# Lut99/RayTracer-3

Measured on AMD Instinct MI355X. Metric: Msamples/sec (pixels x spp) at 1920x1080x512spp, higher is better.
Workload: dtype f32

## Files before the change

include/rt3.h:

```cpp
#ifndef RT3_H
#define RT3_H

#include <stdint.h>

#ifdef __cplusplus
extern "C" {
#endif

#define RT3_ABI_VERSION 3u
uint32_t rt3_abi_version(void);


#define RT3_E_ARG     (-1)
#define RT3_E_DEVICE  (-2)
#define RT3_E_IO      (-3)
#define RT3_E_STATE   (-4)


typedef struct rt3_gface {
    uint32_t v1, v2, v3;
    uint32_t _pad0;
    float    normal[3];
    uint32_t _pad1;
    float    color[3];
// ... 237 lines not shown
uint32_t rt3_scene_weekend(uint32_t seed, float* center_radius, rt3_material* materials, uint32_t cap);
uint32_t rt3_scene_stress(uint32_t n, uint32_t seed, float* center_radius, rt3_material* materials, uint32_t cap);
uint32_t rt3_scene_cornell(uint32_t grid, rt3_gface* faces, float* vertices_xyzw, rt3_material* face_materials,
                           uint32_t cap_faces);

uint32_t rt3_hash_u32(uint32_t x);
float    rt3_random_float(uint32_t m);

int      rt3_debug_force_plain_mode_r(rt3_ctx* ctx, int on);
int      rt3_debug_force_brute(rt3_ctx* ctx, int on);
int      rt3_debug_force_flat_filter(rt3_ctx* ctx, int on);
int      rt3_debug_arith(rt3_ctx* ctx, const float* a, const float* b, uint32_t n, float* div, float* sq, float* fm,
                         float* cs, float* sn, float* sk3, uint32_t* pk);
int      rt3_debug_primary_lists(rt3_ctx* ctx, const rt3_camera* cam, const rt3_params* p, uint32_t* out_masks, uint64_t capacity_words,
                                 uint32_t* n_groups, uint32_t* n_blocks);

#ifdef __cplusplus
}
#endif
#endif
```

raytracer-3_amd/__init__.py:

```python
import ctypes as C
import os

import numpy as np

_HERE = os.path.dirname(os.path.abspath(__file__))
LIB_PATH = os.environ.get("RT3_LIB_PATH", os.path.join(_HERE, "librt3hip.so"))

GFACE = np.dtype([("v1", "<u4"), ("v2", "<u4"), ("v3", "<u4"), ("_p0", "<u4"),
                  ("normal", "<f4", 3), ("_p1", "<u4"), ("color", "<f4", 3), ("_p2", "<u4")])
MATERIAL = np.dtype([("rgb", "<f4", 3), ("param", "<f4"), ("kind", "<u4")])

MAT_FLAT, MAT_LAMBERT, MAT_METAL, MAT_DIELECTRIC = 0, 1, 2, 3
RAY = np.dtype([("origin", "<f4", 3), ("t_max", "<f4"), ("direction", "<f4", 3), ("_pad", "<u4")])
HIT = np.dtype([("t", "<f4"), ("kind", "<u4"), ("index", "<u4"), ("_pad", "<u4")])
HIT_NONE, HIT_FACE, HIT_SPHERE, HIT_INVALID = 0, 1, 2, 3
AOV = np.dtype([("albedo", "<f4", 3), ("coverage", "<f4"), ("normal", "<f4", 3), ("depth", "<f4"), ("kind", "<u4"), ("index", "<u4"),
                ("_pad", "<u4", 2)])
HISTORY = np.dtype([("colour", "<f4", 3), ("length", "<f4"), ("moments", "<f4", 2), ("depth", "<f4"), ("_pad0", "<f4"),
                    ("normal", "<f4", 3), ("_pad1", "<f4")])
OCCLUDED_INVALID = 0xFFFFFFFF
FLAG_GAMMA2, FLAG_BLACK_BACKGROUND, FLAG_REFERENCE_PRIMARY, FLAG_VARIANCE = 1, 2, 4, 8
REGROUP_SPHERES, REGROUP_MESH = 1, 2


# ... 73 lines not shown
    "rt3_render", "rt3_render_device", "rt3_render_path", "rt3_render_path_device", "rt3_rows_owned",
    "rt3_row_of_local", "rt3_get_stats", "rt3_prerender_triangle", "rt3_sphere_face_count",
    "rt3_sphere_vertex_count", "rt3_prerender_sphere", "rt3_object_count", "rt3_prerender_object",
    "rt3_transfer_entity", "rt3_camera_update", "rt3_camera_look_at", "rt3_frame_ppm_bytes", "rt3_frame_to_ppm",
    "rt3_scene_three_spheres", "rt3_scene_weekend", "rt3_scene_stress", "rt3_scene_cornell", "rt3_hash_u32",
    "rt3_random_float", "rt3_debug_arith", "rt3_debug_force_plain_mode_r",
    "rt3_mesh_begin", "rt3_mesh_put", "rt3_mesh_sphere", "rt3_mesh_commit", "rt3_mesh_download",
    "rt3_render_path_range", "rt3_render_path_range_device", "rt3_accum_download", "rt3_accum_upload", "rt3_gather_rows",
    "rt3_stream", "rt3_synchronize", "rt3_device_alloc_words", "rt3_device_free", "rt3_device_read_words", "rt3_debug_force_brute",
    "rt3_abi_version", "rt3_debug_force_flat_filter", "rt3_gather_plan",
    "rt3_intersect", "rt3_occluded", "rt3_intersect_device", "rt3_occluded_device",
    "rt3_camera_rays", "rt3_camera_rays_device", "rt3_render_aov", "rt3_render_aov_device", "rt3_accum_resolve", "rt3_accum_resolve_device",
    "rt3_frame_pfm_bytes", "rt3_frame_to_pfm", "rt3_denoise", "rt3_denoise_device", "rt3_denoise_temporal", "rt3_denoise_temporal_device",
    "rt3_motion", "rt3_motion_device", "rt3_denoise_temporal_motion", "rt3_denoise_temporal_motion_device",
    "rt3_update_spheres", "rt3_update_spheres_device", "rt3_update_mesh", "rt3_update_mesh_device",
    "rt3_debug_primary_lists",
    "rt3_regroup", "rt3_regroup_device", "rt3_debug_group_order",
    "rt3_render_path_adaptive", "rt3_render_path_adaptive_device",
]
ABI_VERSION = 3

_lib = None


def lib():
    global _lib
    if _lib is not None:
        return _lib
    if not os.path.exists(LIB_PATH):
        raise Fatal("librt3hip.so not found at %s — build it with `python -c 'import __graft_entry__ as g; g.build()'`; "
                    "there is no CPU fallback" % LIB_PATH)
# ... 11 lines not shown
        "rt3_render_path": (i32, [vp, vp, vp, vp]), "rt3_render_path_device": (i32, [vp, vp, vp, vp, vp]),
        "rt3_rows_owned": (u32, [vp]), "rt3_row_of_local": (u32, [vp, u32]), "rt3_get_stats": (i32, [vp, vp]),
        "rt3_prerender_triangle": (None, [vp, vp, vp, vp, vp, vp]),
        "rt3_sphere_face_count": (u32, [u32, u32]), "rt3_sphere_vertex_count": (u32, [u32, u32]),
        "rt3_prerender_sphere": (None, [vp, f32, u32, u32, vp, vp, vp]),
        "rt3_object_count": (i32, [C.c_char_p, vp, vp]),
        "rt3_prerender_object": (i32, [C.c_char_p, vp, f32, vp, vp, u32, vp, u32]),
        "rt3_transfer_entity": (None, [vp, vp, vp, vp, vp, u32, vp, u32]),
        "rt3_camera_update": (None, [vp, f32, f32, f32]), "rt3_camera_look_at": (None, [vp, vp, vp, vp, f32, f32, f32]),
        "rt3_frame_ppm_bytes": (u64, [vp, u32, u32, vp, u64]), "rt3_frame_to_ppm": (i32, [vp, u32, u32, C.c_char_p]),
        "rt3_scene_three_spheres": (u32, [vp, vp, u32]), "rt3_scene_weekend": (u32, [u32, vp, vp, u32]),
        "rt3_scene_stress": (u32, [u32, u32, vp, vp, u32]), "rt3_scene_cornell": (u32, [u32, vp, vp, vp, u32]),
        "rt3_hash_u32": (u32, [u32]), "rt3_random_float": (f32, [u32]),
        "rt3_debug_arith": (i32, [vp, vp, vp, u32, vp, vp, vp, vp, vp, vp, vp]),
        "rt3_debug_force_plain_mode_r": (i32, [vp, i32]),
        "rt3_debug_primary_lists": (i32, [vp, vp, vp, vp, u64, vp, vp]),
        "rt3_mesh_begin": (i32, [vp, u32, u32]), "rt3_mesh_put": (i32, [vp, vp, u32, vp, u32, u32, u32]),
        "rt3_mesh_sphere": (i32, [vp, vp, f32, u32, u32, vp, u32, u32]), "rt3_mesh_commit": (i32, [vp, vp]),
        "rt3_mesh_download": (i32, [vp, vp, vp]),
        "rt3_render_path_range": (i32, [vp, vp, vp, u32, u32, vp]),
        "rt3_render_path_range_device": (i32, [vp, vp, vp, u32, u32, vp, vp]),
        "rt3_accum_download": (i32, [vp, vp, vp, vp]), "rt3_accum_upload": (i32, [vp, vp, vp, vp, vp, u32]),
        "rt3_gather_rows": (i32, [vp, vp, vp, vp, vp, vp]), "rt3_stream": (vp, [vp]), "rt3_synchronize": (i32, [vp]),
        "rt3_device_alloc_words": (vp, [vp, u64]), "rt3_device_free": (None, [vp, vp]),
        "rt3_device_read_words": (i32, [vp, vp, u64, vp]), "rt3_debug_force_brute": (i32, [vp, i32]),
        "rt3_abi_version": (u32, []), "rt3_debug_force_flat_filter": (i32, [vp, i32]), "rt3_gather_plan": (i32, [vp, vp]),
        "rt3_intersect": (i32, [vp, vp, u32, f32, vp]), "rt3_occluded": (i32, [vp, vp, u32, f32, vp]),
        "rt3_intersect_device": (i32, [vp, vp, u32, f32, vp, vp]), "rt3_occluded_device": (i32, [vp, vp, u32, f32, vp, vp]),
        "rt3_camera_rays": (i32, [vp, vp, vp, u32, u32, vp]), "rt3_camera_rays_device": (i32, [vp, vp, vp, u32, u32, vp, vp]),
        "rt3_render_aov": (i32, [vp, vp, vp, vp]), "rt3_render_aov_device": (i32, [vp, vp, vp, vp, vp]),
        "rt3_accum_resolve": (i32, [vp, vp]), "rt3_accum_resolve_device": (i32, [vp, vp, vp]),
# ... 735 lines not shown
        return outs


    def debug_primary_lists(self, cam, params):
        ng, nb = C.c_uint32(0), C.c_uint32(0)
        npix = rows_owned(params) * params.width
        out = np.zeros((-(-npix // 64), 16), np.uint32)
        self._check(lib().rt3_debug_primary_lists(self._ctx, C.byref(cam), C.byref(params), _p(out), out.size, C.byref(ng), C.byref(nb)))
        return out.reshape(-1)[:ng.value * nb.value].reshape(ng.value, nb.value).copy()


def initialize_renderer(device=0):
    return HipRenderer(device)


def rows_owned(params):
    return lib().rt3_rows_owned(C.byref(params))


def row_of_local(params, local_row):
    return lib().rt3_row_of_local(C.byref(params), local_row)


def deinterleave(tiles, params_list, height, width):
    frame = np.zeros((height, width), np.uint32)
    for tile, p in zip(tiles, params_list):
        for r in range(tile.shape[0]):
            frame[row_of_local(p, r)] = tile[r]
    return frame
```

raytracer-3_amd/csrc/rt3_device.hip:

```cpp
#include <hip/hip_runtime.h>
#include <hipcub/hipcub.hpp>

#include <algorithm>
#include <cmath>
#include <cstdio>
#include <cstdlib>
#include <cstring>
#include <map>
#include <set>
#include <string>
#include <type_traits>
#include <vector>

#include "rt3.h"

#include "rt3_kernel_common.hpp"
#include "rt3_path.hpp"
#include "rt3_valu_scan.hpp"
#include "rt3_matrix_filter.hpp"
#include "rt3_level_filter.hpp"
#include "rt3_reduce.hpp"
#include "rt3_adaptive.hpp"
#include "rt3_aov.hpp"
#include "rt3_denoise.hpp"
// ... 517 lines not shown
    const bool sph_lds = has_sph && ctx->n_sph <= kSphLdsMax;
    const bool grouped = kGroupTri > 1 && kGroupSph > 1 && (query || (!ctx->force_flat && !getenv("RT3_NO_GROUPS")));
    A.n_tri_rows = grouped ? ctx->tri.n_groups : ctx->n_faces;
    A.n_sph_rows = grouped ? ctx->sph.n_groups : ctx->n_sph;
    A.sph_grp = ctx->sph.grp; A.sph_perm = ctx->sph.perm; A.tri_grp = ctx->tri.grp; A.tri_perm = ctx->tri.perm; A.tri_rec = ctx->d_tri_rec;
    A.tri_leaf = ctx->tri.leaf; A.sph_leaf = ctx->sph.leaf; A.n_tri_leaves = ctx->tri.n_leaves; A.n_sph_leaves = ctx->sph.n_leaves;
    A.tri_rowb = ctx->tri.rowb; A.sph_rowb = ctx->sph.rowb;
    T.mfma_blocks = (ctx->n_sph + 31u) / 32u;
    bool resident = false;
    uint32_t levels = 0;
    if (brute) {
        T.plain = query ? k_trace_brute<false, true> : ref ? k_trace_brute<true> : list ? k_trace_brute<false, false, true> : k_trace_brute<false>;
    } else if (mfma_single) {
        T.lds = single_k64 ? (size_t)T.mfma_blocks * (4096 + 32 * (16 + 16 + 4 + 4)) + (size_t)kBitmapBytes
                           : (size_t)T.mfma_blocks * (2048 + 32 * (16 + 16 + 4 + 4)) + (size_t)kBitmapBytes + (size_t)kMB * 8 + (size_t)(kMB / 64) * kPairCap * 4;
        T.block = kMB;
        T.single = single_k64 ? (list ? k_trace_mfma<true> : k_trace_mfma<>) : query ? k_trace_mfma32<true> : list ? k_trace_mfma32<false, true> : k_trace_mfma32<>;
        T.frag_a = (const u32x4*)(single_k64 ? ctx->d_sph_frag.get() : ctx->d_sph_frag32.get());
        if (!query && !single_k64) {
            T.filter_counted = true;
            const char* on = getenv("RT3_PRIMARY_LISTS"); const char* cap = getenv("RT3_PRIMARY_LIST_MAX");
            A.prim_masks = nullptr;
            A.prim_list_max = 0;
            if (!list && !(on && atoi(on) == 0)) {
                T.list_groups = (A.npix + 63u) / 64u;
                int rc_;
                if ((rc_ = ctx->d_prim_masks.ensure(ctx, (size_t)T.list_groups * T.mfma_blocks))) return rc_;
                A.prim_masks = ctx->d_prim_masks;
                A.prim_list_max = cap ? (uint32_t)std::min<long>(std::max<long>(atol(cap), 0), (long)kMfmaSphMax) : kPrimaryListMax;
            }
// ... 1514 lines not shown
    RT3_HIP(hipEventElapsedTime(&out->total_ms, ctx->ev_begin, ctx->ev_end));
    out->launches = ctx->ev_used;
    out->samples = ctx->last_samples;
    out->n_spheres = ctx->n_sph;
    out->n_faces = ctx->n_faces;
    if (ctx->last_was_path) {
        unsigned long long counters[kCastSlots] = { 0 };
        RT3_HIP(hipMemcpy(counters, ctx->d_casts, sizeof counters, hipMemcpyDeviceToHost));
#ifdef RT3_PROFILE_PHASES
        if (counters[13] != 0) {
            const double all = (double)(counters[11] + counters[12] + counters[13] + counters[14] + counters[15] + counters[17]);
            fprintf(stderr, "[rt3 profile] k_trace_mfma32 / k_trace_mfma, share of wave time: refill %.1f %%, ray operands (+ direct spheres) %.1f %%, scan %.1f %%, "
                            "push + exact tests %.1f %%, decode + shade %.1f %%, restock (primary pass) %.1f %%\n",
                    100.0 * counters[11] / all, 100.0 * counters[12] / all, 100.0 * counters[13] / all, 100.0 * counters[14] / all, 100.0 * counters[15] / all,
                    100.0 * counters[17] / all);
        }
#endif
#ifdef RT3_PROFILE
        if (counters[13] == 0)
        fprintf(stderr, "[rt3 profile] wave iterations %llu, flush iterations/wave-iter %.2f, candidates/ray %.2f, live lanes/wave-iter %.1f, "
                        "fresh paths/wave-iter %.1f\n", counters[4], (double)counters[2] / (double)counters[4],
                (double)counters[3] / (double)counters[0], (double)counters[0] / (double)counters[4], (double)counters[5] / (double)counters[4]);
        if (counters[13] != 0) {
            const double all = (double)(counters[12] + counters[13] + counters[14] + counters[15] + counters[4]);
            fprintf(stderr, "[rt3 profile] tiled kernel, share of wave time: barriers + tile fill %.1f %%, scan %.1f %%, push %.1f %%, exact tests %.1f %%, "
                            "refill / operands / shade %.1f %%\n", 100.0 * counters[12] / all, 100.0 * counters[13] / all, 100.0 * counters[14] / all,
                    100.0 * counters[15] / all, 100.0 * counters[4] / all);
        } else {
        fprintf(stderr, "[rt3 profile] first wave ended %.1f us before the last one\n", (double)(counters[7] - counters[6]) / 100.0);
        fprintf(stderr, "[rt3 profile] timeline from the first wave's start (us): last wave start %.1f, queue first seen empty %.1f, last seen empty %.1f, "
// ... 30 lines not shown
    RT3_HIP(hipMemcpy(da, a, N * 4, hipMemcpyHostToDevice));
    RT3_HIP(hipMemcpy(db, b, N * 4, hipMemcpyHostToDevice));
    hipLaunchKernelGGL(k_debug_arith, dim3((n + 255) / 256), dim3(256), 0, ctx->stream, da, db, n, ddiv, dsq, dfm, dcs, dsn, dsk, dpk);
    RT3_HIP(hipGetLastError());
    RT3_HIP(hipStreamSynchronize(ctx->stream));
    RT3_HIP(hipMemcpy(div, ddiv, N * 4, hipMemcpyDeviceToHost));
    RT3_HIP(hipMemcpy(sq, dsq, N * 4, hipMemcpyDeviceToHost));
    RT3_HIP(hipMemcpy(fm, dfm, N * 4, hipMemcpyDeviceToHost));
    RT3_HIP(hipMemcpy(cs, dcs, N * 4, hipMemcpyDeviceToHost));
    RT3_HIP(hipMemcpy(sn, dsn, N * 4, hipMemcpyDeviceToHost));
    RT3_HIP(hipMemcpy(sk3, dsk, N * 12, hipMemcpyDeviceToHost));
    RT3_HIP(hipMemcpy(pk, dpk, N * 4, hipMemcpyDeviceToHost));
    return 0;
}

int rt3_debug_primary_lists(rt3_ctx* ctx, const rt3_camera* cam, const rt3_params* p, uint32_t* out_masks, uint64_t capacity_words, uint32_t* n_groups,
                            uint32_t* n_blocks) {
    if (!ctx) return RT3_E_ARG;
    if (!cam || !n_groups || !n_blocks) return fail(ctx, RT3_E_ARG, "cam / n_groups / n_blocks is NULL");
    int rc = check_params(ctx, p);
    if (rc) return rc;
    if (ctx->n_sph == 0 || ctx->n_faces != 0 || ctx->n_sph > kMfmaSphMax) return fail(ctx, RT3_E_STATE, "strip lists need a sphere-only scene of <= 512 spheres");
    hipStream_t stream;
    if ((rc = enter(ctx, nullptr, &stream))) return rc;
    const uint32_t npix = rt3_rows_owned(p) * p->width;
    *n_groups = (npix + 63u) / 64u;
    *n_blocks = (ctx->n_sph + 31u) / 32u;
    const size_t words = (size_t)*n_groups * *n_blocks;
    if (!out_masks || capacity_words < words) return fail(ctx, RT3_E_ARG, "out_masks holds fewer than n_groups * n_blocks words");
    if (words == 0) return 0;
// ... 11 lines not shown
```

raytracer-3_amd/csrc/rt3_kernel_common.hpp:

```cpp
#pragma once

namespace {

constexpr int      kBlock       = 256;
constexpr int      kCandSlots   = 16;
constexpr uint32_t kWorkChunk   = 256;
constexpr uint32_t kSphLdsMax   = 2048;
constexpr uint32_t kModeRTile   = 512;

#define kPadSphere make_float4(0.0f, 0.0f, 0.0f, -1e30f)

struct CamDev { float ox, oy, oz, hx, hy, hz, vx, vy, vz, lx, ly, lz; };

__device__ __forceinline__ float fma_(float a, float b, float c) { return __builtin_fmaf(a, b, c); }
__device__ __forceinline__ float dot3(float ax, float ay, float az, float bx, float by, float bz) {
    return ax * bx + ay * by + az * bz;
}
__device__ __forceinline__ float dotf(float ax, float ay, float az, float bx, float by, float bz) {
    return fma_(az, bz, fma_(ay, by, ax * bx));
}
__device__ __forceinline__ uint32_t lane_id() {
    return __builtin_amdgcn_mbcnt_hi(~0u, __builtin_amdgcn_mbcnt_lo(~0u, 0u));
}
__device__ __forceinline__ uint32_t prefix_count(unsigned long long mask) {
    return __builtin_amdgcn_mbcnt_hi((uint32_t)(mask >> 32), __builtin_amdgcn_mbcnt_lo((uint32_t)mask, 0u));
}

struct FastDiv { uint32_t magic, shift; };
__device__ __forceinline__ uint32_t fdiv(uint32_t n, FastDiv f) {
    if (f.shift == 0xFFFFFFFFu) return n;
    const uint32_t q = __umulhi(f.magic, n);
    return (((n - q) >> 1) + q) >> f.shift;
}

__device__ __forceinline__ uint32_t hash_u32(uint32_t x) {
    x += x << 10; x ^= x >> 6; x += x << 3; x ^= x >> 11; x += x << 15;
    return x;
}
__device__ __forceinline__ uint32_t hash2(uint32_t a, uint32_t b) { return hash_u32(a ^ hash_u32(b)); }
__device__ __forceinline__ float u01(uint32_t m) { return __uint_as_float((m & 0x007FFFFFu) | 0x3F800000u) - 1.0f; }
__device__ __forceinline__ float rnd(uint32_t base, uint32_t ctr) { return u01(hash2(base, ctr)); }

__device__ __forceinline__ void sky(float dx, float dy, float dz, float& r, float& g, float& b) {
    const float len = __builtin_sqrtf(dot3(dx, dy, dz, dx, dy, dz));
    const float uy = dy / len;
    const float t = 0.5f * (uy + 1.0f);
    const float a = 1.0f - t;
    r = a * 1.0f + t * 0.5f;
    g = a * 1.0f + t * 0.7f;
    b = a * 1.0f + t * 1.0f;
}
__device__ __forceinline__ uint32_t pack_channel(float c) {
    float m = c < 0.0f ? 0.0f : c;
    m = 1.0f < m ? 1.0f : m;
    return (uint32_t)(__builtin_roundf(m * 255.0f)) & 0xFFu;
}
// ... 110 lines not shown
    const float disc = fma_(h, h, -c);
    if (!((c < 0.0f) | ((disc > 0.0f) & (h > 0.0f)))) return false;
    const float sq = __builtin_sqrtf(disc);
    float t = h - sq;
    if (!(t > t_min)) t = h + sq;
    t_out = t;
    return t > t_min;
}

__device__ __forceinline__ uint32_t frame_row(const TraceArgs& A, uint32_t local_row) {
    if (A.tile_count <= 1) return local_row;
    const uint32_t lb = fdiv(local_row, A.div_tile_rows), in = local_row - lb * A.tile_rows;
    return (lb * A.tile_count + A.tile_index) * A.tile_rows + in;
}

template <bool REF = false, bool LIST = false>
__device__ __forceinline__ void start_path(const TraceArgs& A, uint32_t item, Path& P) {
    const uint32_t sb = fdiv(item, A.div_npix);
    uint32_t pix = item - sb * A.npix;
    if constexpr (LIST) pix = A.active[pix];
    const uint32_t s = A.s0 + sb;
    const uint32_t lrow = fdiv(pix, A.div_width), x = pix - lrow * A.width;
    const uint32_t y = frame_row(A, lrow);
    const uint32_t base = hash2(y * A.width + x, hash2(s, A.seed));
    float jx = 0.0f, jy = 0.0f;
    if (A.spp > 1) {
        const float xi0 = rnd(base, 1), xi1 = rnd(base, 2);
        if (A.edge != 0) {
            const uint32_t sy = fdiv(s, A.div_edge), sx = s - sy * A.edge;
            jx = ((float)sx + xi0) / (float)A.edge - 0.5f;
            jy = ((float)sy + xi1) / (float)A.edge - 0.5f;
        } else { jx = xi0 - 0.5f; jy = xi1 - 0.5f; }
    }
    const float u = ((float)x + jx) / ((float)A.width - 1.0f);
    const float v = ((float)(A.height - 1 - y) + jy) / ((float)A.height - 1.0f);
    const CamDev& c = A.cam;
    float rx = ((c.lx + u * c.hx) + v * c.vx) - c.ox;
    float ry = ((c.ly + u * c.hy) + v * c.vy) - c.oy;
    float rz = ((c.lz + u * c.hz) + v * c.vz) - c.oz;
// ... 6 lines not shown
        const float a = r * cs, b = r * sn;
        const float fx = a * A.lux + b * A.lvx, fy = a * A.luy + b * A.lvy, fz = a * A.luz + b * A.lvz;
        ox = ox + fx; oy = oy + fy; oz = oz + fz;
        rx = rx - fx; ry = ry - fy; rz = rz - fz;
    }
    P.ox = ox; P.oy = oy; P.oz = oz;
    if (REF) { P.dx = rx; P.dy = ry; P.dz = rz; }
    else {
        const float inv = 1.0f / __builtin_sqrtf(dot3(rx, ry, rz, rx, ry, rz));
        P.dx = rx * inv; P.dy = ry * inv; P.dz = rz * inv;
    }
    P.tr = P.tg = P.tb = 1.0f;
    P.lr = P.lg = P.lb = 0.0f;
    P.slot = item; P.base = base; P.depth = 0;
}

}
```

raytracer-3_amd/csrc/rt3_matrix_filter.hpp:

```cpp
#pragma once

namespace {

constexpr int      kMB        = 1024;
constexpr uint32_t kMfmaSphMax = 512;
constexpr uint32_t kBitmapBytes = 16 * kMB * 4;
constexpr float    kFilterEps = 2e-5f;

typedef __bf16 bf16x8 __attribute__((ext_vector_type(8)));
typedef float f32x16 __attribute__((ext_vector_type(16)));
typedef uint32_t u32x4 __attribute__((ext_vector_type(4)));

__host__ __device__ constexpr uint32_t frag_row_of(uint32_t b) { return ((15u - (b & 15u)) & 3u) + 8u * ((15u - (b & 15u)) >> 2) + 4u * (b >> 4); }

__host__ __device__ inline uint32_t bf16_rn(float x) {
    uint32_t u = __builtin_bit_cast(uint32_t, x);
    u += 0x7FFFu + ((u >> 16) & 1u);
    return u >> 16;
}
__host__ __device__ inline float bf16_up(uint32_t h) { return __builtin_bit_cast(float, h << 16); }
__host__ __device__ inline void split3(float x, uint32_t* parts ) {
    parts[0] = bf16_rn(x);
    const float r1 = x - bf16_up(parts[0]);
    parts[1] = bf16_rn(r1);
// ... 641 lines not shown
        atomicAdd(A.cast_counter + 11, ph_refill); atomicAdd(A.cast_counter + 12, ph_operands); atomicAdd(A.cast_counter + 13, ph_scan);
        atomicAdd(A.cast_counter + 14, ph_flush); atomicAdd(A.cast_counter + 15, ph_shade);
    }
#endif
#undef RT3_SPHASE
    if (lane == 0 && casts != 0) { atomicAdd(A.cast_counter, casts); atomicAdd(A.cast_counter + 1, iters * n_blocks * 8ull); }
#ifdef RT3_PROFILE
    if (lane == 0) {
        atomicAdd(A.cast_counter + 2, prof_flush_iters); atomicAdd(A.cast_counter + 3, prof_cands); atomicAdd(A.cast_counter + 4, iters); atomicAdd(A.cast_counter + 5, prof_refills);
        const unsigned long long now = wall_clock64();
        atomicMin(A.cast_counter + 6, now); atomicMax(A.cast_counter + 7, now);
    }
#endif
}

struct SphereMirror { const float4* sph; const float* invr; const float4* mat; const uint32_t* kind; uint32_t n_blocks; };
template <bool LIST = false>
__device__ __forceinline__ void refill_from_traced_stock(const TraceArgs& A, const SphereMirror& S, uint32_t lane, bool& alive, Path& P, TracedStock& Q,
                                                         uint32_t& chunk_next, uint32_t& chunk_end, bool& exhausted, unsigned long long& casts,
                                                         unsigned long long& exact, unsigned long long& ph_restock) {
    const unsigned long long need = __ballot(!alive);
    if (need == 0ull) return;
    const uint32_t n_need = (uint32_t)__popcll(need), rank = prefix_count(need);
    uint32_t served = 0;
    for (;;) {
        const uint32_t k = min(Q.n, n_need - served);
        if (k != 0) {
            const bool take = !alive && rank >= served && rank < served + k;
            stock_pop(Q, Q.n - 1u - (rank - served), take, P, alive);
            Q.n -= k;
            served += k;
        }
        if (served == n_need || exhausted) return;
        if (chunk_next == chunk_end) {
            uint32_t b = 0;
            if (lane == 0) b = atomicAdd(A.work_counter, kWorkChunk);
            b = __builtin_amdgcn_readfirstlane(b);
            if (b >= A.total) { exhausted = true; return; }
            chunk_next = b;
            chunk_end = min(b + kWorkChunk, A.total);
        }
#ifdef RT3_PROFILE_PHASES
        const unsigned long long ph_t0 = clock64();
#endif
        const uint32_t n_new = min(64u, chunk_end - chunk_next);
        const uint32_t item = min(chunk_next + lane, chunk_end - 1u);
        bool live = lane < n_new;
        Path T;
        start_path<false, LIST>(A, item, T);
        chunk_next += n_new;
        uint32_t word = 0, listed = 0xFFFFFFFFu;
        if (A.prim_masks != nullptr) {
            const uint32_t grp = (item - fdiv(item, A.div_npix) * A.npix) >> 6;
            unsigned long long rest = __ballot(live);
            while (rest != 0ull) {
                const uint32_t g = (uint32_t)__builtin_amdgcn_readlane((int)grp, (int)(__ffsll((long long)rest) - 1));
                if (lane < S.n_blocks) word |= A.prim_masks[(size_t)g * S.n_blocks + lane];
                rest &= ~__ballot(grp == g);
            }
            listed = 0;
            for (uint32_t b = 0; b < S.n_blocks; b++) listed += (uint32_t)__popc((uint32_t)__builtin_amdgcn_readlane((int)word, (int)b));
        }
        if (listed <= A.prim_list_max) {
            casts += n_new;
            unsigned long long key = direct_tests(A, T.ox, T.oy, T.oz, T.dx, T.dy, T.dz, [&](uint32_t j) { return S.sph[j]; });
            for (uint32_t b = 0; b < S.n_blocks; b++) {
                uint32_t m = (uint32_t)__builtin_amdgcn_readlane((int)word, (int)b);
                while (m != 0u) {
                    const uint32_t j = b * 32u + ((uint32_t)__ffs((int)m) - 1u);
                    m &= m - 1u;
                    float t;
                    if (sphere_root(S.sph[j], T.ox, T.oy, T.oz, T.dx, T.dy, T.dz, A.t_min, t) && t < __builtin_inff()) {
                        const unsigned long long kk = hit_key(t, 1u, j);
                        key = kk < key ? kk : key;
                    }
                    exact += n_new;
                }
            }
            uint32_t kind, ibest;
            float tbest;
            key_decode(key, kind, ibest, tbest);
            shade_lane<false, true>(A, T, live, kind, ibest, tbest, S.sph, S.invr, S.mat, S.kind);
            const unsigned long long surv = __ballot(live);
            const uint32_t n = (uint32_t)__popcll(surv), before = prefix_count(surv);
            const int to = (int)((live ? before : n + (lane - before)) * 4u);
            auto send = [&](uint32_t v) { return (uint32_t)__builtin_amdgcn_ds_permute(to, (int)v); };
            auto sendf = [&](float v) { return __uint_as_float(send(__float_as_uint(v))); };
            Q.ox = sendf(T.ox); Q.oy = sendf(T.oy); Q.oz = sendf(T.oz); Q.dx = sendf(T.dx); Q.dy = sendf(T.dy); Q.dz = sendf(T.dz);
            Q.tr = sendf(T.tr); Q.tg = sendf(T.tg); Q.tb = sendf(T.tb);
            Q.slot = send(T.slot); Q.base = send(T.base); Q.depth = send(T.depth);
            Q.n = n;
        } else {
            Q.ox = T.ox; Q.oy = T.oy; Q.oz = T.oz; Q.dx = T.dx; Q.dy = T.dy; Q.dz = T.dz; Q.slot = T.slot; Q.base = T.base;
            Q.tr = Q.tg = Q.tb = 1.0f; Q.depth = 0;
            Q.n = n_new;
        }
#ifdef RT3_PROFILE_PHASES
        ph_restock += clock64() - ph_t0;
#endif
    }
}

template <bool QUERY = false, bool LIST = false>
__global__ __launch_bounds__(kMB) void k_trace_mfma32(const TraceArgs A, const u32x4* __restrict__ frags, uint32_t n_blocks) {
    extern __shared__ u32x4 lds_dyn[];
    u32x4* s_frag = lds_dyn;
    float4* s_sph = reinterpret_cast<float4*>(s_frag + (size_t)n_blocks * 128);
    float4* s_mat = s_sph + (size_t)n_blocks * 32;
    float* s_invr = reinterpret_cast<float*>(s_mat + (size_t)n_blocks * 32);
    uint32_t* s_kind = reinterpret_cast<uint32_t*>(s_invr + (size_t)n_blocks * 32);
    uint32_t* s_bm = reinterpret_cast<uint32_t*>(s_kind + (size_t)n_blocks * 32);
    unsigned long long* s_key = reinterpret_cast<unsigned long long*>(s_bm + 16 * kMB);
    uint32_t* s_pairs = reinterpret_cast<uint32_t*>(s_key + kMB);
    const uint32_t tid = threadIdx.x, lane = lane_id();
    uint32_t* pairs = s_pairs + (tid / 64u) * kPairCap;
    unsigned long long* keys = s_key + (tid & ~63u);
    for (uint32_t k = tid; k < n_blocks * 128; k += kMB) s_frag[k] = frags[k];
    for (uint32_t k = tid; k < n_blocks * 32; k += kMB) {
        const bool in = k < A.n_sph;
        s_sph[k] = in ? A.sph[k] : kPadSphere;
        s_mat[k] = in ? A.sph_mat[k] : make_float4(0.0f, 0.0f, 0.0f, 0.0f);
        s_invr[k] = in ? A.sph_invr[k] : 0.0f;
        s_kind[k] = in ? A.sph_kind[k] : 0u;
    }
    __syncthreads();

    Path P;
    P.ox = P.oy = P.oz = 0.0f; P.dx = P.dy = 0.0f; P.dz = 1.0f;
    P.tr = P.tg = P.tb = 0.0f; P.lr = P.lg = P.lb = 0.0f; P.slot = 0; P.base = 0; P.depth = 0; P.tmax = __builtin_inff();
    bool alive = false;
    uint32_t chunk_next = 0, chunk_end = 0;
    bool exhausted = false;
    TracedStock Q;
    Q.ox = Q.oy = Q.oz = 0.0f; Q.dx = Q.dy = 0.0f; Q.dz = 1.0f; Q.tr = Q.tg = Q.tb = 0.0f; Q.slot = 0; Q.base = 0; Q.depth = 0; Q.n = 0;
    const SphereMirror mirror = { s_sph, s_invr, s_mat, s_kind, n_blocks };
    unsigned long long casts = 0, iters = 0, exact = 0;
    unsigned long long primary_casts = 0, ph_restock = 0;
#ifdef RT3_PROFILE_PHASES
    unsigned long long ph_refill = 0, ph_operands = 0, ph_scan = 0, ph_flush = 0, ph_shade = 0, ph_mark = clock64();
#define RT3_SPHASE(acc) { const unsigned long long now_ = clock64(); acc += now_ - ph_mark; ph_mark = now_; }
#else
#define RT3_SPHASE(acc)
#endif

    for (;;) {
        if constexpr (QUERY) refill_queries(A, lane, alive, P, chunk_next, chunk_end, exhausted);
        else refill_from_traced_stock<LIST>(A, mirror, lane, alive, P, Q, chunk_next, chunk_end, exhausted, primary_casts, exact, ph_restock);
        RT3_SPHASE(ph_refill)
        const unsigned long long live = __ballot(alive);
        if (live == 0ull) break;
        casts += (unsigned long long)__popcll(live);
        iters++;
// ... 13 lines not shown
            float t;
            if (sphere_root(s_sph[j], r.ox, r.oy, r.oz, r.dx, r.dy, r.dz, A.t_min, t) && t < __builtin_inff()) atomicMin(&keys[src], hit_key(t, 1u, j));
        };
        RT3_SPHASE(ph_operands)
        const uint32_t nz = mfma32k_scan_tile<kMB, false>(s_frag, n_blocks, R, s_bm + tid, lane);
        RT3_SPHASE(ph_scan)
        push_pairs16<kMB, RT3_DECODE_FP6 != 0>(nz, n_blocks, s_bm + tid, 0u, lane, pairs, n_pairs, test);
        test_all_raw<RT3_DECODE_FP6 != 0>(lane, pairs, n_pairs, test);
        RT3_SPHASE(ph_flush)
        __builtin_amdgcn_wave_barrier();
        uint32_t kind, ibest;
        float tbest;
        if constexpr (QUERY) query_sink(A, P, alive, keys[lane]);
        else {
            key_decode(keys[lane], kind, ibest, tbest);
            shade_lane<false, true>(A, P, alive, kind, ibest, tbest, s_sph, s_invr, s_mat, s_kind);
        }
        RT3_SPHASE(ph_shade)
    }
#ifdef RT3_PROFILE_PHASES
    if (lane == 0) {
        atomicAdd(A.cast_counter + 11, ph_refill - ph_restock); atomicAdd(A.cast_counter + 12, ph_operands); atomicAdd(A.cast_counter + 13, ph_scan);
        atomicAdd(A.cast_counter + 14, ph_flush); atomicAdd(A.cast_counter + 15, ph_shade); atomicAdd(A.cast_counter + 17, ph_restock);
    }
#endif
#undef RT3_SPHASE
    if constexpr (QUERY) {
        if (lane == 0 && casts != 0) { atomicAdd(A.cast_counter, casts); atomicAdd(A.cast_counter + 1, iters * n_blocks * 8ull); atomicAdd(A.cast_counter + 2, exact); }
    } else if (lane == 0 && casts + primary_casts != 0) {
        atomicAdd(A.cast_counter, casts + primary_casts); atomicAdd(A.cast_counter + 1, iters * n_blocks * 8ull); atomicAdd(A.cast_counter + 2, exact);
        atomicAdd(A.cast_counter + 16, casts);
    }
}

#ifndef RT3_TILED_TB
#define RT3_TILED_TB 1024
#endif
#ifndef RT3_TILE_LOADS
// ... 445 lines not shown
```

raytracer-3_amd/csrc/rt3_path.hpp:

```cpp
#pragma once

namespace {

__device__ __forceinline__ void query_store(const TraceArgs& A, uint32_t slot, uint32_t kind, uint32_t idx, float t) {
    if (A.q_occluded) reinterpret_cast<uint32_t*>(A.q_out)[slot] = kind == RT3_HIT_INVALID ? 0xFFFFFFFFu : (kind != RT3_HIT_NONE ? 1u : 0u);
    else reinterpret_cast<uint4*>(A.q_out)[slot] = make_uint4(__float_as_uint(t), kind, idx, 0u);
}
__device__ __forceinline__ bool query_ray(const TraceArgs& A, uint32_t item, Path& P) {
    const float4* r = A.q_rays + 2 * (size_t)item;
    const float4 a = r[0], b = r[1];
    P.ox = a.x; P.oy = a.y; P.oz = a.z; P.tmax = a.w;
    P.dx = b.x; P.dy = b.y; P.dz = b.z;
    P.slot = item; P.depth = 0;
    const float dd = dotf(b.x, b.y, b.z, b.x, b.y, b.z);
    const bool finite = __builtin_isfinite(a.x) & __builtin_isfinite(a.y) & __builtin_isfinite(a.z) &
                        __builtin_isfinite(b.x) & __builtin_isfinite(b.y) & __builtin_isfinite(b.z);
    const bool ok = finite && __builtin_fabsf(dd - 1.0f) <= 0x1p-20f && a.w > A.t_min;
    if (!ok) query_store(A, item, RT3_HIT_INVALID, 0xFFFFFFFFu, __builtin_nanf(""));
    return ok;
}

template <bool REF = false, bool QUERY = false, bool LIST = false>
__device__ __forceinline__ void refill_lanes(const TraceArgs& A, uint32_t lane, bool& alive, Path& P, uint32_t& chunk_next,
                                             uint32_t& chunk_end, bool& exhausted) {
// ... 73 lines not shown
}

struct TracedStock { float ox, oy, oz, dx, dy, dz, tr, tg, tb; uint32_t slot, base, depth; uint32_t n; };
__device__ __forceinline__ void stock_pop(const TracedStock& Q, uint32_t src, bool take, Path& P, bool& alive) {
    const int s = (int)src;
    const float ox = __shfl(Q.ox, s), oy = __shfl(Q.oy, s), oz = __shfl(Q.oz, s), dx = __shfl(Q.dx, s), dy = __shfl(Q.dy, s), dz = __shfl(Q.dz, s);
    const float tr = __shfl(Q.tr, s), tg = __shfl(Q.tg, s), tb = __shfl(Q.tb, s);
    const uint32_t slot = (uint32_t)__shfl((int)Q.slot, s), base = (uint32_t)__shfl((int)Q.base, s), depth = (uint32_t)__shfl((int)Q.depth, s);
    if (take) {
        P.ox = ox; P.oy = oy; P.oz = oz; P.dx = dx; P.dy = dy; P.dz = dz; P.slot = slot; P.base = base;
        P.tr = tr; P.tg = tg; P.tb = tb; P.lr = P.lg = P.lb = 0.0f; P.depth = depth;
        alive = true;
    }
}

template <bool HAS_TRI, bool HAS_SPH, bool REF = false>
__device__ __forceinline__ void shade_lane(const TraceArgs& A, Path& P, bool& alive, uint32_t kind, uint32_t ibest, float tbest,
                                           const float4* sph, const float* sph_invr, const float4* sph_mat, const uint32_t* sph_kind) {
    const float ox = P.ox, oy = P.oy, oz = P.oz;
    float dx = P.dx, dy = P.dy, dz = P.dz;
    if (alive) {
        bool done = false;
        if (kind == 0) {
            if (!(A.flags & RT3_FLAG_BLACK_BACKGROUND)) {
                float r, g, b;
                sky(dx, dy, dz, r, g, b);
                P.lr = fma_(P.tr, r, P.lr); P.lg = fma_(P.tg, g, P.lg); P.lb = fma_(P.tb, b, P.lb);
            }
            done = true;
        } else {
            float4 m; uint32_t mk;
            float px, py, pz, nx, ny, nz;
            if (HAS_TRI && (!HAS_SPH || kind == 1)) {
// ... 9 lines not shown
                nx = (px - s.x) * invr; ny = (py - s.y) * invr; nz = (pz - s.z) * invr;
            }
            if (mk == RT3_MAT_FLAT) {
                P.lr = fma_(P.tr, m.x, P.lr); P.lg = fma_(P.tg, m.y, P.lg); P.lb = fma_(P.tb, m.z, P.lb);
                done = true;
            } else if (P.depth + 1 == A.max_depth) {
                done = true;
            } else {
                if (REF && P.depth == 0) {
                    const float inv = 1.0f / __builtin_sqrtf(dot3(dx, dy, dz, dx, dy, dz));
                    dx = dx * inv; dy = dy * inv; dz = dz * inv;
                }
                const bool front = dotf(dx, dy, dz, nx, ny, nz) < 0.0f;
                if (!front) { nx = -nx; ny = -ny; nz = -nz; }
                const uint32_t ctr = 1u + 8u * (P.depth + 1u);
                float sx, sy, sz;
                float ar = m.x, ag = m.y, ab = m.z;
                const float dn = dotf(dx, dy, dz, nx, ny, nz);
                float vx = 0.0f, vy = 0.0f, vz = 0.0f;
                if ((mk == RT3_MAT_LAMBERT) | ((mk == RT3_MAT_METAL) & (m.w > 0.0f)))
                    unit_vector(rnd(P.base, ctr), rnd(P.base, ctr + 1), vx, vy, vz);
                const float k2 = 2.0f * dn;
                const float mx = fma_(-k2, nx, dx), my = fma_(-k2, ny, dy), mz = fma_(-k2, nz, dz);
                if (mk == RT3_MAT_LAMBERT) {
                    sx = nx + vx; sy = ny + vy; sz = nz + vz;
                    if (__builtin_fabsf(sx) < 1e-8f && __builtin_fabsf(sy) < 1e-8f && __builtin_fabsf(sz) < 1e-8f) { sx = nx; sy = ny; sz = nz; }
                } else if (mk == RT3_MAT_METAL) {
                    const float inv = 1.0f / __builtin_sqrtf(dotf(mx, my, mz, mx, my, mz));
                    const float rx = mx * inv, ry = my * inv, rz = mz * inv;
                    sx = rx; sy = ry; sz = rz;
                    if (m.w > 0.0f) { sx = fma_(m.w, vx, rx); sy = fma_(m.w, vy, ry); sz = fma_(m.w, vz, rz); }
                    if (!(dotf(sx, sy, sz, nx, ny, nz) > 0.0f)) done = true;
                } else {
                    const float ri = front ? m.x : m.w;
                    float cosv = -dn;
                    if (cosv > 1.0f) cosv = 1.0f;
                    const float s2 = fma_(-cosv, cosv, 1.0f);
                    const float sinv = __builtin_sqrtf(s2 > 0.0f ? s2 : 0.0f);
                    const bool cannot = ri * sinv > 1.0f;
                    const float r0 = front ? m.y : m.z;
                    const float xx = 1.0f - cosv, x2 = xx * xx, x5 = x2 * x2 * xx;
                    const float R = fma_(1.0f - r0, x5, r0);
                    if (cannot || R > rnd(P.base, ctr + 2)) {
                        sx = mx; sy = my; sz = mz;
                    } else {
                        const float ex = fma_(cosv, nx, dx) * ri, ey = fma_(cosv, ny, dy) * ri, ez = fma_(cosv, nz, dz) * ri;
                        const float par = -__builtin_sqrtf(__builtin_fabsf(1.0f - dotf(ex, ey, ez, ex, ey, ez)));
                        sx = fma_(par, nx, ex); sy = fma_(par, ny, ey); sz = fma_(par, nz, ez);
                    }
                    ar = ag = ab = 1.0f;
                }
                if (!done) {
                    const float inv = 1.0f / __builtin_sqrtf(dotf(sx, sy, sz, sx, sy, sz));
                    P.dx = sx * inv; P.dy = sy * inv; P.dz = sz * inv;
                    P.ox = px; P.oy = py; P.oz = pz;
                    P.tr *= ar; P.tg *= ag; P.tb *= ab;
                    P.depth += 1;
                }
// ... 11 lines not shown
```

Before: 12920.

## Precompute per-depth hash table and exploit wave-uniform sample/group in restock

```diff
diff --git a/include/rt3.h b/include/rt3.h
--- a/include/rt3.h
+++ b/include/rt3.h
@@ -275,6 +275,7 @@
                          float* cs, float* sn, float* sk3, uint32_t* pk);
 int      rt3_debug_primary_lists(rt3_ctx* ctx, const rt3_camera* cam, const rt3_params* p, uint32_t* out_masks, uint64_t capacity_words,
                                  uint32_t* n_groups, uint32_t* n_blocks);
+uint32_t rt3_debug_ctr_table(uint32_t* out, uint32_t capacity_rows);
 
 #ifdef __cplusplus
 }
diff --git a/raytracer-3_amd/__init__.py b/raytracer-3_amd/__init__.py
--- a/raytracer-3_amd/__init__.py
+++ b/raytracer-3_amd/__init__.py
@@ -111,7 +111,7 @@
     "rt3_frame_pfm_bytes", "rt3_frame_to_pfm", "rt3_denoise", "rt3_denoise_device", "rt3_denoise_temporal", "rt3_denoise_temporal_device",
     "rt3_motion", "rt3_motion_device", "rt3_denoise_temporal_motion", "rt3_denoise_temporal_motion_device",
     "rt3_update_spheres", "rt3_update_spheres_device", "rt3_update_mesh", "rt3_update_mesh_device",
-    "rt3_debug_primary_lists",
+    "rt3_debug_primary_lists", "rt3_debug_ctr_table",
     "rt3_regroup", "rt3_regroup_device", "rt3_debug_group_order",
     "rt3_render_path_adaptive", "rt3_render_path_adaptive_device",
 ]
@@ -153,7 +153,7 @@
         "rt3_hash_u32": (u32, [u32]), "rt3_random_float": (f32, [u32]),
         "rt3_debug_arith": (i32, [vp, vp, vp, u32, vp, vp, vp, vp, vp, vp, vp]),
         "rt3_debug_force_plain_mode_r": (i32, [vp, i32]),
-        "rt3_debug_primary_lists": (i32, [vp, vp, vp, vp, u64, vp, vp]),
+        "rt3_debug_primary_lists": (i32, [vp, vp, vp, vp, u64, vp, vp]), "rt3_debug_ctr_table": (u32, [vp, u32]),
         "rt3_mesh_begin": (i32, [vp, u32, u32]), "rt3_mesh_put": (i32, [vp, vp, u32, vp, u32, u32, u32]),
         "rt3_mesh_sphere": (i32, [vp, vp, f32, u32, u32, vp, u32, u32]), "rt3_mesh_commit": (i32, [vp, vp]),
         "rt3_mesh_download": (i32, [vp, vp, vp]),
@@ -919,6 +919,13 @@
     return HipRenderer(device)
 
 
+def debug_ctr_table():
+    rows = lib().rt3_debug_ctr_table(None, 0)
+    out = np.zeros((rows, 4), np.uint32)
+    lib().rt3_debug_ctr_table(_p(out), rows)
+    return out
+
+
 def rows_owned(params):
     return lib().rt3_rows_owned(C.byref(params))
 
diff --git a/raytracer-3_amd/csrc/rt3_device.hip b/raytracer-3_amd/csrc/rt3_device.hip
--- a/raytracer-3_amd/csrc/rt3_device.hip
+++ b/raytracer-3_amd/csrc/rt3_device.hip
@@ -555,6 +555,7 @@
     } else if (mfma_single) {
         T.lds = single_k64 ? (size_t)T.mfma_blocks * (4096 + 32 * (16 + 16 + 4 + 4)) + (size_t)kBitmapBytes
                            : (size_t)T.mfma_blocks * (2048 + 32 * (16 + 16 + 4 + 4)) + (size_t)kBitmapBytes + (size_t)kMB * 8 + (size_t)(kMB / 64) * kPairCap * 4;
+        if (!single_k64 && !query && RT3_CTR_TABLE) T.lds += kCtrTableBytes;
         T.block = kMB;
         T.single = single_k64 ? (list ? k_trace_mfma<true> : k_trace_mfma<>) : query ? k_trace_mfma32<true> : list ? k_trace_mfma32<false, true> : k_trace_mfma32<>;
         T.frag_a = (const u32x4*)(single_k64 ? ctx->d_sph_frag.get() : ctx->d_sph_frag32.get());
@@ -2099,6 +2100,10 @@
                             "push + exact tests %.1f %%, decode + shade %.1f %%, restock (primary pass) %.1f %%\n",
                     100.0 * counters[11] / all, 100.0 * counters[12] / all, 100.0 * counters[13] / all, 100.0 * counters[14] / all, 100.0 * counters[15] / all,
                     100.0 * counters[17] / all);
+            if (counters[17] != 0)
+                fprintf(stderr, "[rt3 profile] restock, share of its wave time: ray generation %.1f %%, list fetch %.1f %%, direct + listed tests %.1f %%, "
+                                "shade %.1f %%, compaction %.1f %%\n", 100.0 * counters[18] / counters[17], 100.0 * counters[19] / counters[17],
+                        100.0 * counters[20] / counters[17], 100.0 * counters[21] / counters[17], 100.0 * counters[22] / counters[17]);
         }
 #endif
 #ifdef RT3_PROFILE
@@ -2159,6 +2164,11 @@
     return 0;
 }
 
+uint32_t rt3_debug_ctr_table(uint32_t* out, uint32_t capacity_rows) {
+    if (out) for (uint32_t k = 0; k < std::min(capacity_rows, kCtrDepthCap) * 4u; k++) out[k] = ctr_table_word(k);
+    return kCtrDepthCap;
+}
+
 int rt3_debug_primary_lists(rt3_ctx* ctx, const rt3_camera* cam, const rt3_params* p, uint32_t* out_masks, uint64_t capacity_words, uint32_t* n_groups,
                             uint32_t* n_blocks) {
     if (!ctx) return RT3_E_ARG;
diff --git a/raytracer-3_amd/csrc/rt3_kernel_common.hpp b/raytracer-3_amd/csrc/rt3_kernel_common.hpp
--- a/raytracer-3_amd/csrc/rt3_kernel_common.hpp
+++ b/raytracer-3_amd/csrc/rt3_kernel_common.hpp
@@ -33,13 +33,16 @@
     return (((n - q) >> 1) + q) >> f.shift;
 }
 
-__device__ __forceinline__ uint32_t hash_u32(uint32_t x) {
+__host__ __device__ __forceinline__ uint32_t hash_u32(uint32_t x) {
     x += x << 10; x ^= x >> 6; x += x << 3; x ^= x >> 11; x += x << 15;
     return x;
 }
 __device__ __forceinline__ uint32_t hash2(uint32_t a, uint32_t b) { return hash_u32(a ^ hash_u32(b)); }
 __device__ __forceinline__ float u01(uint32_t m) { return __uint_as_float((m & 0x007FFFFFu) | 0x3F800000u) - 1.0f; }
 __device__ __forceinline__ float rnd(uint32_t base, uint32_t ctr) { return u01(hash2(base, ctr)); }
+constexpr uint32_t kCtrDepthCap = 64;
+constexpr uint32_t kCtrTableBytes = kCtrDepthCap * 16;
+__host__ __device__ __forceinline__ uint32_t ctr_table_word(uint32_t k) { return hash_u32(1u + 8u * ((k >> 2) + 1u) + (k & 3u)); }
 
 __device__ __forceinline__ void sky(float dx, float dy, float dz, float& r, float& g, float& b) {
     const float len = __builtin_sqrtf(dot3(dx, dy, dz, dx, dy, dz));
@@ -180,15 +183,9 @@
     return (lb * A.tile_count + A.tile_index) * A.tile_rows + in;
 }
 
-template <bool REF = false, bool LIST = false>
-__device__ __forceinline__ void start_path(const TraceArgs& A, uint32_t item, Path& P) {
-    const uint32_t sb = fdiv(item, A.div_npix);
-    uint32_t pix = item - sb * A.npix;
-    if constexpr (LIST) pix = A.active[pix];
-    const uint32_t s = A.s0 + sb;
-    const uint32_t lrow = fdiv(pix, A.div_width), x = pix - lrow * A.width;
-    const uint32_t y = frame_row(A, lrow);
-    const uint32_t base = hash2(y * A.width + x, hash2(s, A.seed));
+template <bool REF = false, bool HS = false>
+__device__ __forceinline__ void start_path_at(const TraceArgs& A, uint32_t item, uint32_t s, uint32_t x, uint32_t y, uint32_t hs, Path& P) {
+    const uint32_t base = hash2(y * A.width + x, HS ? hs : hash2(s, A.seed));
     float jx = 0.0f, jy = 0.0f;
     if (A.spp > 1) {
         const float xi0 = rnd(base, 1), xi1 = rnd(base, 2);
@@ -225,5 +222,15 @@
     P.lr = P.lg = P.lb = 0.0f;
     P.slot = item; P.base = base; P.depth = 0;
 }
-
-}
+template <bool REF = false, bool LIST = false>
+__device__ __forceinline__ void start_path(const TraceArgs& A, uint32_t item, Path& P) {
+    const uint32_t sb = fdiv(item, A.div_npix);
+    uint32_t pix = item - sb * A.npix;
+    if constexpr (LIST) pix = A.active[pix];
+    const uint32_t s = A.s0 + sb;
+    const uint32_t lrow = fdiv(pix, A.div_width), x = pix - lrow * A.width;
+    const uint32_t y = frame_row(A, lrow);
+    start_path_at<REF>(A, item, s, x, y, 0u, P);
+}
+
+}
diff --git a/raytracer-3_amd/csrc/rt3_matrix_filter.hpp b/raytracer-3_amd/csrc/rt3_matrix_filter.hpp
--- a/raytracer-3_amd/csrc/rt3_matrix_filter.hpp
+++ b/raytracer-3_amd/csrc/rt3_matrix_filter.hpp
@@ -679,11 +679,27 @@
 #endif
 }
 
-struct SphereMirror { const float4* sph; const float* invr; const float4* mat; const uint32_t* kind; uint32_t n_blocks; };
+#ifndef RT3_CTR_TABLE
+#define RT3_CTR_TABLE 1
+#endif
+#ifndef RT3_UNIFORM_SAMPLE
+#define RT3_UNIFORM_SAMPLE 1
+#endif
+#ifndef RT3_UNIFORM_GROUP
+#define RT3_UNIFORM_GROUP 1
+#endif
+#ifndef RT3_COMPACT_SKIP
+#define RT3_COMPACT_SKIP 1
+#endif
+static_assert(kMfmaSphMax / 32u <= 32u, "refill_from_traced_stock keeps one bit per row block in a 32-bit word (blocks)");
+typedef const __attribute__((address_space(4))) uint32_t* ConstWords;
+__device__ __forceinline__ uint32_t uniform(uint32_t v) { return (uint32_t)__builtin_amdgcn_readfirstlane((int)v); }
+struct RestockPhases { unsigned long long total = 0, raygen = 0, fetch = 0, tests = 0, shade = 0, compact = 0; };
+struct SphereMirror { const float4* sph; const float* invr; const float4* mat; const uint32_t* kind; uint32_t n_blocks; const uint4* ctr_tab; };
 template <bool LIST = false>
 __device__ __forceinline__ void refill_from_traced_stock(const TraceArgs& A, const SphereMirror& S, uint32_t lane, bool& alive, Path& P, TracedStock& Q,
                                                          uint32_t& chunk_next, uint32_t& chunk_end, bool& exhausted, unsigned long long& casts,
-                                                         unsigned long long& exact, unsigned long long& ph_restock) {
+                                                         unsigned long long& exact, RestockPhases& ph) {
     const unsigned long long need = __ballot(!alive);
     if (need == 0ull) return;
     const uint32_t n_need = (uint32_t)__popcll(need), rank = prefix_count(need);
@@ -707,62 +723,122 @@
         }
 #ifdef RT3_PROFILE_PHASES
         const unsigned long long ph_t0 = clock64();
+        unsigned long long ph_mark = ph_t0;
+#define RT3_RPHASE(acc) { const unsigned long long now_ = clock64(); acc += now_ - ph_mark; ph_mark = now_; }
+#else
+#define RT3_RPHASE(acc)
 #endif
         const uint32_t n_new = min(64u, chunk_end - chunk_next);
         const uint32_t item = min(chunk_next + lane, chunk_end - 1u);
         bool live = lane < n_new;
         Path T;
-        start_path<false, LIST>(A, item, T);
+        constexpr bool kFirstItem = !LIST && (RT3_UNIFORM_SAMPLE || RT3_UNIFORM_GROUP);
+        uint32_t pix0 = 0, s_first = 0;
+        bool one_sample = false;
+        if constexpr (kFirstItem) {
+            const uint32_t first = uniform(chunk_next), sb0 = uniform(fdiv(first, A.div_npix));
+            one_sample = sb0 == uniform(fdiv(first + (n_new - 1u), A.div_npix));
+            pix0 = first - sb0 * A.npix;
+            s_first = A.s0 + sb0;
+        }
+        const uint32_t step = min(lane, n_new - 1u);
+        if (!LIST && RT3_UNIFORM_SAMPLE && one_sample) {
+            const uint32_t hs = uniform(hash2(s_first, A.seed));
+            const uint32_t lrow0 = uniform(fdiv(pix0, A.div_width)), x0 = pix0 - lrow0 * A.width;
+            uint32_t x = x0 + step, lrow = lrow0;
+            while (__ballot(x >= A.width) != 0ull)
+                if (x >= A.width) { x -= A.width; lrow += 1u; }
+            start_path_at<false, true>(A, item, s_first, x, frame_row(A, lrow), hs, T);
+        } else start_path<false, LIST>(A, item, T);
         chunk_next += n_new;
-        uint32_t word = 0, listed = 0xFFFFFFFFu;
+        RT3_RPHASE(ph.raygen)
+        uint32_t word = 0, listed = 0xFFFFFFFFu, blocks = 0;
+        const bool one_group = !LIST && RT3_UNIFORM_GROUP && one_sample && (pix0 >> 6) == ((pix0 + (n_new - 1u)) >> 6);
+        ConstWords tab = nullptr;
         if (A.prim_masks != nullptr) {
-            const uint32_t grp = (item - fdiv(item, A.div_npix) * A.npix) >> 6;
-            unsigned long long rest = __ballot(live);
-            while (rest != 0ull) {
-                const uint32_t g = (uint32_t)__builtin_amdgcn_readlane((int)grp, (int)(__ffsll((long long)rest) - 1));
-                if (lane < S.n_blocks) word |= A.prim_masks[(size_t)g * S.n_blocks + lane];
-                rest &= ~__ballot(grp == g);
+            listed = 0;
+            if (one_group) {
+                tab = (ConstWords)(A.prim_masks + (size_t)(pix0 >> 6) * S.n_blocks);
+#pragma unroll 4
+                for (uint32_t b = 0; b < S.n_blocks; b++) {
+                    const uint32_t w = tab[b];
+                    listed += (uint32_t)__popc(w);
+                    blocks |= (w != 0u ? 1u : 0u) << b;
+                }
+            } else {
+                const uint32_t grp = (kFirstItem && one_sample ? pix0 + step : item - fdiv(item, A.div_npix) * A.npix) >> 6;
+                unsigned long long rest = __ballot(live);
+                while (rest != 0ull) {
+                    const uint32_t g = (uint32_t)__builtin_amdgcn_readlane((int)grp, (int)(__ffsll((long long)rest) - 1));
+                    if (lane < S.n_blocks) word |= A.prim_masks[(size_t)g * S.n_blocks + lane];
+                    rest &= ~__ballot(grp == g);
+                }
+                for (uint32_t b = 0; b < S.n_blocks; b++) listed += (uint32_t)__popc((uint32_t)__builtin_amdgcn_readlane((int)word, (int)b));
             }
-            listed = 0;
-            for (uint32_t b = 0; b < S.n_blocks; b++) listed += (uint32_t)__popc((uint32_t)__builtin_amdgcn_readlane((int)word, (int)b));
-        }
+        }
+        RT3_RPHASE(ph.fetch)
         if (listed <= A.prim_list_max) {
             casts += n_new;
             unsigned long long key = direct_tests(A, T.ox, T.oy, T.oz, T.dx, T.dy, T.dz, [&](uint32_t j) { return S.sph[j]; });
-            for (uint32_t b = 0; b < S.n_blocks; b++) {
-                uint32_t m = (uint32_t)__builtin_amdgcn_readlane((int)word, (int)b);
-                while (m != 0u) {
-                    const uint32_t j = b * 32u + ((uint32_t)__ffs((int)m) - 1u);
-                    m &= m - 1u;
-                    float t;
-                    if (sphere_root(S.sph[j], T.ox, T.oy, T.oz, T.dx, T.dy, T.dz, A.t_min, t) && t < __builtin_inff()) {
-                        const unsigned long long kk = hit_key(t, 1u, j);
-                        key = kk < key ? kk : key;
+            auto listed_sphere = [&](uint32_t j) {
+                float t;
+                if (sphere_root(S.sph[j], T.ox, T.oy, T.oz, T.dx, T.dy, T.dz, A.t_min, t) && t < __builtin_inff()) {
+                    const unsigned long long kk = hit_key(t, 1u, j);
+                    key = kk < key ? kk : key;
+                }
+                exact += n_new;
+            };
+            if (one_group) {
+                while (blocks != 0u) {
+                    const uint32_t b = (uint32_t)__ffs((int)blocks) - 1u;
+                    blocks &= blocks - 1u;
+                    uint32_t m = tab[b];
+                    while (m != 0u) {
+                        listed_sphere(b * 32u + ((uint32_t)__ffs((int)m) - 1u));
+                        m &= m - 1u;
                     }
-                    exact += n_new;
+                }
+            } else {
+                for (uint32_t b = 0; b < S.n_blocks; b++) {
+                    uint32_t m = (uint32_t)__builtin_amdgcn_readlane((int)word, (int)b);
+                    while (m != 0u) {
+                        listed_sphere(b * 32u + ((uint32_t)__ffs((int)m) - 1u));
+                        m &= m - 1u;
+                    }
                 }
             }
+            RT3_RPHASE(ph.tests)
             uint32_t kind, ibest;
             float tbest;
             key_decode(key, kind, ibest, tbest);
-            shade_lane<false, true>(A, T, live, kind, ibest, tbest, S.sph, S.invr, S.mat, S.kind);
+            shade_lane<false, true, false, RT3_CTR_TABLE != 0>(A, T, live, kind, ibest, tbest, S.sph, S.invr, S.mat, S.kind, S.ctr_tab);
+            RT3_RPHASE(ph.shade)
             const unsigned long long surv = __ballot(live);
-            const uint32_t n = (uint32_t)__popcll(surv), before = prefix_count(surv);
-            const int to = (int)((live ? before : n + (lane - before)) * 4u);
-            auto send = [&](uint32_t v) { return (uint32_t)__builtin_amdgcn_ds_permute(to, (int)v); };
-            auto sendf = [&](float v) { return __uint_as_float(send(__float_as_uint(v))); };
-            Q.ox = sendf(T.ox); Q.oy = sendf(T.oy); Q.oz = sendf(T.oz); Q.dx = sendf(T.dx); Q.dy = sendf(T.dy); Q.dz = sendf(T.dz);
-            Q.tr = sendf(T.tr); Q.tg = sendf(T.tg); Q.tb = sendf(T.tb);
-            Q.slot = send(T.slot); Q.base = send(T.base); Q.depth = send(T.depth);
+            const uint32_t n = (uint32_t)__popcll(surv);
+            if (RT3_COMPACT_SKIP && (n == 0u || n == 64u)) {
+                Q.ox = T.ox; Q.oy = T.oy; Q.oz = T.oz; Q.dx = T.dx; Q.dy = T.dy; Q.dz = T.dz;
+                Q.tr = T.tr; Q.tg = T.tg; Q.tb = T.tb;
+                Q.slot = T.slot; Q.base = T.base; Q.depth = T.depth;
+            } else {
+                const uint32_t before = prefix_count(surv);
+                const int to = (int)((live ? before : n + (lane - before)) * 4u);
+                auto send = [&](uint32_t v) { return (uint32_t)__builtin_amdgcn_ds_permute(to, (int)v); };
+                auto sendf = [&](float v) { return __uint_as_float(send(__float_as_uint(v))); };
+                Q.ox = sendf(T.ox); Q.oy = sendf(T.oy); Q.oz = sendf(T.oz); Q.dx = sendf(T.dx); Q.dy = sendf(T.dy); Q.dz = sendf(T.dz);
+                Q.tr = sendf(T.tr); Q.tg = sendf(T.tg); Q.tb = sendf(T.tb);
+                Q.slot = send(T.slot); Q.base = send(T.base); Q.depth = send(T.depth);
+            }
             Q.n = n;
+            RT3_RPHASE(ph.compact)
         } else {
             Q.ox = T.ox; Q.oy = T.oy; Q.oz = T.oz; Q.dx = T.dx; Q.dy = T.dy; Q.dz = T.dz; Q.slot = T.slot; Q.base = T.base;
             Q.tr = Q.tg = Q.tb = 1.0f; Q.depth = 0;
             Q.n = n_new;
         }
 #ifdef RT3_PROFILE_PHASES
-        ph_restock += clock64() - ph_t0;
-#endif
+        ph.total += clock64() - ph_t0;
+#endif
+#undef RT3_RPHASE
     }
 }
 
@@ -777,9 +853,12 @@
     uint32_t* s_bm = reinterpret_cast<uint32_t*>(s_kind + (size_t)n_blocks * 32);
     unsigned long long* s_key = reinterpret_cast<unsigned long long*>(s_bm + 16 * kMB);
     uint32_t* s_pairs = reinterpret_cast<uint32_t*>(s_key + kMB);
+    constexpr bool CTR = !QUERY && RT3_CTR_TABLE != 0;
+    uint32_t* s_ctr = s_pairs + (kMB / 64u) * kPairCap;
     const uint32_t tid = threadIdx.x, lane = lane_id();
     uint32_t* pairs = s_pairs + (tid / 64u) * kPairCap;
     unsigned long long* keys = s_key + (tid & ~63u);
+    if constexpr (CTR) for (uint32_t k = tid; k < kCtrDepthCap * 4u; k += kMB) s_ctr[k] = ctr_table_word(k);
     for (uint32_t k = tid; k < n_blocks * 128; k += kMB) s_frag[k] = frags[k];
     for (uint32_t k = tid; k < n_blocks * 32; k += kMB) {
         const bool in = k < A.n_sph;
@@ -798,9 +877,11 @@
     bool exhausted = false;
     TracedStock Q;
     Q.ox = Q.oy = Q.oz = 0.0f; Q.dx = Q.dy = 0.0f; Q.dz = 1.0f; Q.tr = Q.tg = Q.tb = 0.0f; Q.slot = 0; Q.base = 0; Q.depth = 0; Q.n = 0;
-    const SphereMirror mirror = { s_sph, s_invr, s_mat, s_kind, n_blocks };
+    const uint4* ctr_tab = reinterpret_cast<const uint4*>(s_ctr);
+    const SphereMirror mirror = { s_sph, s_invr, s_mat, s_kind, n_blocks, ctr_tab };
     unsigned long long casts = 0, iters = 0, exact = 0;
-    unsigned long long primary_casts = 0, ph_restock = 0;
+    unsigned long long primary_casts = 0;
+    RestockPhases ph_restock;
 #ifdef RT3_PROFILE_PHASES
     unsigned long long ph_refill = 0, ph_operands = 0, ph_scan = 0, ph_flush = 0, ph_shade = 0, ph_mark = clock64();
 #define RT3_SPHASE(acc) { const unsigned long long now_ = clock64(); acc += now_ - ph_mark; ph_mark = now_; }
@@ -844,14 +925,16 @@
         if constexpr (QUERY) query_sink(A, P, alive, keys[lane]);
         else {
             key_decode(keys[lane], kind, ibest, tbest);
-            shade_lane<false, true>(A, P, alive, kind, ibest, tbest, s_sph, s_invr, s_mat, s_kind);
+            shade_lane<false, true, false, CTR>(A, P, alive, kind, ibest, tbest, s_sph, s_invr, s_mat, s_kind, ctr_tab);
         }
         RT3_SPHASE(ph_shade)
     }
 #ifdef RT3_PROFILE_PHASES
     if (lane == 0) {
-        atomicAdd(A.cast_counter + 11, ph_refill - ph_restock); atomicAdd(A.cast_counter + 12, ph_operands); atomicAdd(A.cast_counter + 13, ph_scan);
-        atomicAdd(A.cast_counter + 14, ph_flush); atomicAdd(A.cast_counter + 15, ph_shade); atomicAdd(A.cast_counter + 17, ph_restock);
+        atomicAdd(A.cast_counter + 11, ph_refill - ph_restock.total); atomicAdd(A.cast_counter + 12, ph_operands); atomicAdd(A.cast_counter + 13, ph_scan);
+        atomicAdd(A.cast_counter + 14, ph_flush); atomicAdd(A.cast_counter + 15, ph_shade); atomicAdd(A.cast_counter + 17, ph_restock.total);
+        atomicAdd(A.cast_counter + 18, ph_restock.raygen); atomicAdd(A.cast_counter + 19, ph_restock.fetch); atomicAdd(A.cast_counter + 20, ph_restock.tests);
+        atomicAdd(A.cast_counter + 21, ph_restock.shade); atomicAdd(A.cast_counter + 22, ph_restock.compact);
     }
 #endif
 #undef RT3_SPHASE
diff --git a/raytracer-3_amd/csrc/rt3_path.hpp b/raytracer-3_amd/csrc/rt3_path.hpp
--- a/raytracer-3_amd/csrc/rt3_path.hpp
+++ b/raytracer-3_amd/csrc/rt3_path.hpp
@@ -111,9 +111,10 @@
     }
 }
 
-template <bool HAS_TRI, bool HAS_SPH, bool REF = false>
+template <bool HAS_TRI, bool HAS_SPH, bool REF = false, bool CTR = false>
 __device__ __forceinline__ void shade_lane(const TraceArgs& A, Path& P, bool& alive, uint32_t kind, uint32_t ibest, float tbest,
-                                           const float4* sph, const float* sph_invr, const float4* sph_mat, const uint32_t* sph_kind) {
+                                           const float4* sph, const float* sph_invr, const float4* sph_mat, const uint32_t* sph_kind,
+                                           const uint4* ctr_tab = nullptr) {
     const float ox = P.ox, oy = P.oy, oz = P.oz;
     float dx = P.dx, dy = P.dy, dz = P.dz;
     if (alive) {
@@ -153,12 +154,18 @@
                 const bool front = dotf(dx, dy, dz, nx, ny, nz) < 0.0f;
                 if (!front) { nx = -nx; ny = -ny; nz = -nz; }
                 const uint32_t ctr = 1u + 8u * (P.depth + 1u);
+                uint32_t h0 = 0, h1 = 0, h2 = 0;
+                if constexpr (CTR) {
+                    if (P.depth < kCtrDepthCap) { const uint4 row = ctr_tab[P.depth]; h0 = row.x; h1 = row.y; h2 = row.z; }
+                    else { h0 = hash_u32(ctr); h1 = hash_u32(ctr + 1u); h2 = hash_u32(ctr + 2u); }
+                }
+                auto xi = [&](uint32_t k, uint32_t h) { return CTR ? u01(hash_u32(P.base ^ h)) : rnd(P.base, ctr + k); };
                 float sx, sy, sz;
                 float ar = m.x, ag = m.y, ab = m.z;
                 const float dn = dotf(dx, dy, dz, nx, ny, nz);
                 float vx = 0.0f, vy = 0.0f, vz = 0.0f;
                 if ((mk == RT3_MAT_LAMBERT) | ((mk == RT3_MAT_METAL) & (m.w > 0.0f)))
-                    unit_vector(rnd(P.base, ctr), rnd(P.base, ctr + 1), vx, vy, vz);
+                    unit_vector(xi(0, h0), xi(1, h1), vx, vy, vz);
                 const float k2 = 2.0f * dn;
                 const float mx = fma_(-k2, nx, dx), my = fma_(-k2, ny, dy), mz = fma_(-k2, nz, dz);
                 if (mk == RT3_MAT_LAMBERT) {
@@ -180,7 +187,7 @@
                     const float r0 = front ? m.y : m.z;
                     const float xx = 1.0f - cosv, x2 = xx * xx, x5 = x2 * x2 * xx;
                     const float R = fma_(1.0f - r0, x5, r0);
-                    if (cannot || R > rnd(P.base, ctr + 2)) {
+                    if (cannot || R > xi(2, h2)) {
                         sx = mx; sy = my; sz = mz;
                     } else {
                         const float ex = fma_(cosv, nx, dx) * ri, ey = fma_(cosv, ny, dy) * ri, ez = fma_(cosv, nz, dz) * ri;
```

Result: faster. 13190 (median of 6 runs) (+2.1%).
